# byuccl/coast

Measured on NVIDIA H100. Metric: protected-kernel throughput (MB/s voted output), sha256 TMR, higher is better.
Workload: dtype u32

## Files before the change

### coast_b200/csrc/coast_rt.c

```c
#define _GNU_SOURCE
#include "../../include/coast_rt.h"
#include "xmr_args.h"
#include "xmr_geom.h"

#include <cuda.h>
#include <ctype.h>
#include <dlfcn.h>
#include <sched.h>
#include <stdarg.h>
#include <stdio.h>
#include <stdlib.h>
#include <string.h>
#include <sys/syscall.h>
#include <unistd.h>

extern const unsigned char coast_kernels_cubin[];

__attribute__((weak)) uint32_t TMR_ERROR_CNT = 0;
__attribute__((weak)) uint64_t __SYNC_COUNT = 0;
__attribute__((weak)) void FAULT_DETECTED_DWC(void) {
    fprintf(stderr, "coast_rt: DWC mismatch detected -> FAULT_DETECTED_DWC -> abort()\n");
    abort();
}

#define DRV_FUNCS(X)                                                                                         \
    X(cuInit, (unsigned int))                                                                                \
    X(cuDeviceGet, (CUdevice*, int))                                                                         \
    X(cuDeviceGetAttribute, (int*, CUdevice_attribute, CUdevice))                                            \
    X(cuDeviceGetPCIBusId, (char*, int, CUdevice))                                                           \
    X(cuPointerGetAttribute, (void*, CUpointer_attribute, CUdeviceptr))                                      \
    X(cuDevicePrimaryCtxRetain, (CUcontext*, CUdevice))                                                      \
    X(cuDevicePrimaryCtxRelease_v2, (CUdevice))                                                              \
    X(cuCtxSetCurrent, (CUcontext))                                                                          \
    X(cuCtxGetCurrent, (CUcontext*))                                                                         \
    X(cuModuleLoadData, (CUmodule*, const void*))                                                            \
    X(cuModuleUnload, (CUmodule))                                                                            \
    X(cuModuleGetFunction, (CUfunction*, CUmodule, const char*))                                             \
    X(cuFuncSetAttribute, (CUfunction, CUfunction_attribute, int))                                           \
    X(cuOccupancyMaxActiveBlocksPerMultiprocessor, (int*, CUfunction, int, size_t))                          \
    X(cuLaunchKernel, (CUfunction, unsigned, unsigned, unsigned, unsigned, unsigned, unsigned, unsigned,     \
                       CUstream, void**, void**))                                                            \
    X(cuMemAlloc_v2, (CUdeviceptr*, size_t))                                                                 \
    X(cuMemFree_v2, (CUdeviceptr))                                                                           \
    X(cuMemPoolCreate, (CUmemoryPool*, const CUmemPoolProps*))                                               \
    X(cuMemPoolDestroy, (CUmemoryPool))                                                                      \
    X(cuMemPoolSetAttribute, (CUmemoryPool, CUmemPool_attribute, void*))                                     \
    X(cuMemAllocFromPoolAsync, (CUdeviceptr*, size_t, CUmemoryPool, CUstream))                               \
    X(cuMemFreeAsync, (CUdeviceptr, CUstream))                                                               \
    X(cuMemcpyHtoDAsync_v2, (CUdeviceptr, const void*, size_t, CUstream))                                    \
    X(cuMemcpyDtoHAsync_v2, (void*, CUdeviceptr, size_t, CUstream))                                          \
    X(cuMemcpyDtoDAsync_v2, (CUdeviceptr, CUdeviceptr, size_t, CUstream))                                    \
    X(cuMemsetD8Async, (CUdeviceptr, unsigned char, size_t, CUstream))                                       \
    X(cuMemHostAlloc, (void**, size_t, unsigned int))                                                        \
    X(cuMemFreeHost, (void*))                                                                                \
    X(cuStreamCreate, (CUstream*, unsigned int))                                                             \
    X(cuStreamDestroy_v2, (CUstream))                                                                        \
    X(cuStreamSynchronize, (CUstream))                                                                       \
    X(cuEventCreate, (CUevent*, unsigned int))                                                               \
    X(cuEventRecord, (CUevent, CUstream))                                                                    \
    X(cuEventDestroy_v2, (CUevent))                                                                          \
    X(cuStreamWaitEvent, (CUstream, CUevent, unsigned int))                                                  \
    X(cuGetErrorString, (CUresult, const char**))                                                            \
    X(cuIpcGetMemHandle, (CUipcMemHandle*, CUdeviceptr))                                                     \
    X(cuIpcOpenMemHandle_v2, (CUdeviceptr*, CUipcMemHandle, unsigned int))                                   \
    X(cuIpcCloseMemHandle, (CUdeviceptr))                                                                    \
    X(cuTensorMapEncodeTiled, (CUtensorMap*, CUtensorMapDataType, cuuint32_t, void*, const cuuint64_t*,      \
                               const cuuint64_t*, const cuuint32_t*, const cuuint32_t*, CUtensorMapInterleave, \
                               CUtensorMapSwizzle, CUtensorMapL2promotion, CUtensorMapFloatOOBfill))

#define X(name, args) static CUresult(CUDAAPI* p_##name) args;
DRV_FUNCS(X)
#undef X

typedef struct {
    uintptr_t base;
    cuuint64_t dim[3], stride[2];
    cuuint32_t box[3], rank;
    CUtensorMapDataType dtype;
    CUtensorMapSwizzle swz;
    CUtensorMapL2promotion l2;
    int in_scratch;
} map_desc;
_Static_assert(sizeof(map_desc) == 80, "map_desc has no padding");

typedef struct { CUdeviceptr p; size_t cap; } dev_buf;
typedef struct { CUstream s; dev_buf in, out, aux, stat, rows, sc; } host_slot;

#define MAX_FN 128
static struct {
    int inited;
    void* libcuda;
    int device;
    CUdevice dev;
    CUcontext ctx;
    CUmodule mod;
    int sm_count;
    CUdeviceptr counters;
    CUdeviceptr peer_counters;
    uint64_t* h_counters;
    struct { char name[64]; CUfunction fn; int ctas_per_sm; unsigned smem; } fns[MAX_FN];
    int n_fns;
    char err[512];
    uint32_t def_nc, def_flags; int def_set;
    host_slot slot[3];
    dev_buf h_b; CUevent ev_b;
    CUmemoryPool pool;
    int numa_node;
    int busy;
    struct { map_desc key; CUtensorMap map; } tmaps[16];
    int n_tmaps, tmap_next;
    unsigned warned_store_votes;
    int host_path_default;
    const char* last_host_path;
} G;

static int enter(void);
static void leave(void) { __atomic_store_n(&G.busy, 0, __ATOMIC_RELEASE); }

static int fail(int code, const char* fmt, ...) {
    va_list ap; va_start(ap, fmt);
    vsnprintf(G.err, sizeof G.err, fmt, ap);
    va_end(ap);
    return code;
}
static int enter(void) {
    if (__atomic_exchange_n(&G.busy, 1, __ATOMIC_ACQUIRE)) {
        return COAST_ERR_BUSY;
    }
    return COAST_OK;
}
#define ENTER() do { int e_ = enter(); if (e_) return e_; } while (0)
#define LEAVE(rc) do { int l_ = (rc); leave(); return l_; } while (0)
static int drv_fail(CUresult r, const char* what) {
    const char* s = NULL;
    if (p_cuGetErrorString) p_cuGetErrorString(r, &s);
    return fail(-(int)r, "%s: CUDA error %d (%s)", what, (int)r, s ? s : "?");
}
#define DRV(call) do { CUresult r_ = (call); if (r_ != CUDA_SUCCESS) return drv_fail(r_, #call); } while (0)

const char* coast_last_error(void) { return G.err; }
const char* coast_version(void) { return "coast_rt 0.1 (sm_90a)"; }

static int bind_driver(void) {
    if (G.libcuda) return COAST_OK;
    void* h = dlopen("libcuda.so.1", RTLD_NOW | RTLD_GLOBAL);
    if (!h) h = dlopen("libcuda.so", RTLD_NOW | RTLD_GLOBAL);
    if (!h) return fail(COAST_ERR_NO_DRIVER, "libcuda.so.1 not found (%s): no GPU driver on this machine; "
                                              "libcoast_rt has no CPU fallback", dlerror());
#define X(name, args)                                                                 \
    *(void**)(&p_##name) = dlsym(h, #name);                                           \
    if (!p_##name) { dlclose(h); return fail(COAST_ERR_NO_DRIVER, "libcuda lacks %s", #name); }
    DRV_FUNCS(X)
#undef X
    G.libcuda = h;
    return COAST_OK;
}


#ifndef MPOL_PREFERRED
#define MPOL_PREFERRED 1
#endif
static int parse_cpulist(const char* s, cpu_set_t* set) {
    int n = 0;
    CPU_ZERO(set);
    while (*s) {
        while (*s == ',' || isspace((unsigned char)*s)) ++s;
        if (!isdigit((unsigned char)*s)) break;
        char* e; long a = strtol(s, &e, 10), b = a;
        if (*e == '-') b = strtol(e + 1, &e, 10);
        for (long c = a; c <= b && c < CPU_SETSIZE; ++c) { CPU_SET((int)c, set); ++n; }
        s = e;
    }
    return n;
}
static void numa_bind_to_gpu(void) {
    G.numa_node = -1;
    const char* env = getenv("COAST_NUMA_BIND");
    if (env && !strcmp(env, "0")) return;
    char bdf[32] = {0}, path[128], buf[4096];
    if (p_cuDeviceGetPCIBusId(bdf, (int)sizeof bdf - 1, G.dev) != CUDA_SUCCESS) return;
    for (char* c = bdf; *c; ++c) *c = (char)tolower((unsigned char)*c);
    snprintf(path, sizeof path, "/sys/bus/pci/devices/%s/numa_node", bdf);
    FILE* f = fopen(path, "r"); if (!f) return;
    int node = -1; if (fscanf(f, "%d", &node) != 1) node = -1; fclose(f);
    if (node < 0 || node >= 1024) return;
    snprintf(path, sizeof path, "/sys/devices/system/node/node%d/cpulist", node);
    f = fopen(path, "r"); if (!f) return;
    size_t got = fread(buf, 1, sizeof buf - 1, f); fclose(f); buf[got] = 0;
    cpu_set_t want, cur, both;
    if (!parse_cpulist(buf, &want)) return;
    if (sched_getaffinity(0, sizeof cur, &cur)) return;
    CPU_AND(&both, &want, &cur);
    if (!CPU_COUNT(&both)) return;
    if (sched_setaffinity(0, sizeof both, &both)) return;
    unsigned long mask[16]; memset(mask, 0, sizeof mask);
    mask[node / (8 * sizeof(unsigned long))] |= 1ul << (node % (8 * sizeof(unsigned long)));
    syscall(SYS_set_mempolicy, MPOL_PREFERRED, mask, (unsigned long)(8 * sizeof mask));
    G.numa_node = node;
}
int coast_numa_node(void) { return G.inited ? G.numa_node : -1; }

static int ensure_ctx(void) {
    if (!G.inited) return fail(COAST_ERR_NOT_INIT, "coast_init() has not been called");
    CUcontext cur = NULL;
    p_cuCtxGetCurrent(&cur);
    if (cur != G.ctx) DRV(p_cuCtxSetCurrent(G.ctx));
// ... 213 lines not shown
    return kernel == COAST_K_QSORT ? unit_bytes : coast_out_bytes_per_unit(kernel);
}
static uint64_t in_bytes_per_unit(const coast_launch_desc* d) {
    if (!known_kernel(d->kernel)) return 0;
    return KINFO[d->kernel].in_bytes == IN_UNIT_BYTES ? d->unit_bytes : KINFO[d->kernel].in_bytes;
}
static uint64_t aux_bytes_per_unit(const coast_launch_desc* d) {
    return known_kernel(d->kernel) && (d->mode & COAST_AES_KEY_PER_UNIT) ? KINFO[d->kernel].key_bytes : 0;
}

static int encode_map(const map_desc* want, CUdeviceptr scratch, int cached, CUtensorMap* map) {
    map_desc m = *want;
    if (m.in_scratch) { m.base += scratch; m.in_scratch = 0; }
    if (cached)
        for (int i = 0; i < G.n_tmaps; ++i)
            if (!memcmp(&G.tmaps[i].key, &m, sizeof m)) { *map = G.tmaps[i].map; return COAST_OK; }
    static const cuuint32_t estr[3] = { 1, 1, 1 };
    DRV(p_cuTensorMapEncodeTiled(map, m.dtype, m.rank, (void*)m.base, m.dim, m.stride, m.box, estr, CU_TENSOR_MAP_INTERLEAVE_NONE,
                                 m.swz, m.l2, CU_TENSOR_MAP_FLOAT_OOB_FILL_NONE));
    if (cached) {
        const int n_slots = (int)(sizeof G.tmaps / sizeof G.tmaps[0]);
        int k = G.n_tmaps < n_slots ? G.n_tmaps++ : (G.tmap_next++ % n_slots);
        G.tmaps[k].key = m; G.tmaps[k].map = *map;
    }
    return COAST_OK;
}

typedef struct {
    unsigned es;
    int batched, grouped, bt;
    uint64_t P;
    uint64_t rows;
    int b_rows_k;
    uint32_t b_rows;
    int scaled, rowwise;
} mm_shape;

typedef struct launch_plan launch_plan;
struct launch_plan {
    char name[64];
    unsigned block, smem;
    uint64_t ctas;
    unsigned waves;
    unsigned cluster;
    int n_maps, cache_maps;
    map_desc map[2];
    size_t scratch;
    size_t scratch_per_cta;
    int scratch_as_aux;
    int (*prepass)(const launch_plan* L, const coast_launch_desc* d, CUdeviceptr scratch, CUstream s);
    mm_shape mm;
    size_t grp_off;
    unsigned grp_tm, grp_tiles_n;
};

static void plan_ring(launch_plan* L, xmr_args* a, unsigned tile_rows, unsigned row_bytes, unsigned pack, CUtensorMapSwizzle swz) {
    L->ctas = (a->n_units + tile_rows - 1) / tile_rows;
    L->waves = 1;
    a->n_tiles = (unsigned)L->ctas;
    L->n_maps = 1; L->cache_maps = 1;
    map_desc* m = &L->map[0];
    m->dtype = CU_TENSOR_MAP_DATA_TYPE_UINT32; m->rank = 2; m->base = (uintptr_t)a->in;
    m->dim[0] = m->box[0] = (row_bytes << pack) / 4u;
    m->dim[1] = a->n_units >> pack;
    m->stride[0] = row_bytes << pack;
    m->box[1] = (tile_rows / xmr_ring_loads(tile_rows)) >> pack;
    m->swz = swz; m->l2 = CU_TENSOR_MAP_L2_PROMOTION_L2_128B;
}

static void plan_wg_map(map_desc* m, CUtensorMapDataType dtype, unsigned esize, uintptr_t base, int in_scratch, uint32_t K,
                        uint32_t rows, unsigned planes, unsigned box_rows) {
    m->dtype = dtype; m->rank = planes > 1 ? 3 : 2; m->base = base; m->in_scratch = in_scratch;
    m->dim[0] = K; m->dim[1] = rows; m->dim[2] = planes;
    m->stride[0] = (cuuint64_t)K * esize; m->stride[1] = (cuuint64_t)rows * K * esize;
    m->box[0] = 128u / esize; m->box[1] = box_rows; m->box[2] = planes;
    m->swz = CU_TENSOR_MAP_SWIZZLE_128B; m->l2 = CU_TENSOR_MAP_L2_PROMOTION_L2_256B;
}

static int mm_rows_fit(const mm_shape* m) { return m->rows < (1ull << 31) && m->P * m->b_rows < (1ull << 31); }

static int mm_bit_refused(const coast_launch_desc* d, uint32_t bit) {
    if (!(d->mode & bit) || is_matmul(d->kernel)) return COAST_OK;
    const char* what = bit == COAST_MM_BATCHED ? "COAST_MM_BATCHED: batched products exist"
                     : bit == COAST_MM_GROUPED ? "COAST_MM_GROUPED: grouped products exist" : "COAST_MM_B_TRANSPOSED: a transposed B exists";
    return fail(COAST_ERR_BAD_ARG, "%s for MM_U32, GEMM_TF32 and GEMM_BF16 only, plus GEMM_FP8 (kernel %u)", what, d->kernel);
}
static int mm_scale_check(const coast_launch_desc* d) {
    const uint32_t bits = d->mode & (COAST_MM_SCALE_TENSOR | COAST_MM_SCALE_ROWWISE);
    if (!bits) return COAST_OK;
    const char* what = bits == COAST_MM_SCALE_TENSOR ? "COAST_MM_SCALE_TENSOR" : "COAST_MM_SCALE_ROWWISE";
    if (d->kernel != COAST_K_GEMM_FP8)
        return fail(COAST_ERR_BAD_ARG, "%s: scaled products exist for GEMM_FP8 only (kernel %u)",
                    bits == (COAST_MM_SCALE_TENSOR | COAST_MM_SCALE_ROWWISE) ? "COAST_MM_SCALE_TENSOR / COAST_MM_SCALE_ROWWISE" : what, d->kernel);
    if (bits == (COAST_MM_SCALE_TENSOR | COAST_MM_SCALE_ROWWISE))
        return fail(COAST_ERR_BAD_ARG, "COAST_MM_SCALE_TENSOR and COAST_MM_SCALE_ROWWISE cannot be combined: one scale layout per launch");
    if (!d->d_scale_a || !d->d_scale_b)
        return fail(COAST_ERR_BAD_ARG, "%s: d_scale_a and d_scale_b must point to the scales of A and B", what);
    if (((uintptr_t)d->d_scale_a) & 3u) return fail(COAST_ERR_BAD_ARG, "%s: d_scale_a must be 4-byte aligned", what);
    if (bits == COAST_MM_SCALE_ROWWISE && (((uintptr_t)d->d_scale_b) & 7u))
        return fail(COAST_ERR_BAD_ARG, "COAST_MM_SCALE_ROWWISE: d_scale_b must be 8-byte aligned (column scales are read in pairs)");
    return COAST_OK;
}
static int mm_check(const coast_launch_desc* d, mm_shape* m) {
    int rc;
    memset(m, 0, sizeof *m);
    if ((rc = mm_bit_refused(d, COAST_MM_BATCHED)) || (rc = mm_bit_refused(d, COAST_MM_GROUPED)) ||
// ... 106 lines not shown
                                           "4..4096 (got %u)", d->unit_bytes);
        if ((((uintptr_t)d->d_in) & 3u) || (((uintptr_t)d->d_out) & 3u))
            return fail(COAST_ERR_BAD_ARG, "COAST_UNIT_OFFSETS: quicksort's d_in and d_out must be 4-byte aligned");
    }
    if (d->n_units >= (1ull << 32)) return fail(COAST_ERR_BAD_ARG, "COAST_UNIT_OFFSETS: n_units must be below 2^32");
    if (!d->d_aux || (((uintptr_t)d->d_aux) & 7u))
        return fail(COAST_ERR_BAD_ARG, "COAST_UNIT_OFFSETS: d_aux must point to n_units + 1 8-byte aligned uint64_t offsets");
    return COAST_OK;
}

static int prepass_ragged(const launch_plan* L, const coast_launch_desc* d, CUdeviceptr scratch, CUstream s) {
    (void)L;
    DRV(p_cuMemsetD8Async(scratch, 0, XMR_RAGGED_PERM, s));
    const void* off = d->d_aux;
    unsigned long long n = d->n_units;
    unsigned int bound = d->unit_bytes;
    unsigned int kind = d->kernel == COAST_K_SHA256 ? XMR_RAGGED_COST_SHA : d->kernel == COAST_K_QSORT ? XMR_RAGGED_COST_QSORT
                                                                                                       : XMR_RAGGED_COST_CRC;
    const uint64_t ctas = (n + XMR_CTA_THREADS - 1) / XMR_CTA_THREADS, cap = (uint64_t)G.sm_count * 8u;
    const unsigned grid = (unsigned)(ctas < cap ? ctas : cap);
    void* params[] = { &off, &n, &bound, &kind, &scratch };
    int rc = launch_small("xmr_ragged_hist", grid, XMR_CTA_THREADS, params, s); if (rc) return rc;
    void* params_scan[] = { &off, &scratch };
    rc = launch_small("xmr_ragged_scan", 1, XMR_RAGGED_SCAN_THREADS, params_scan, s); if (rc) return rc;
    return launch_small("xmr_ragged_scatter", grid, XMR_CTA_THREADS, params, s);
}

static int run_plan(const launch_plan* L, const coast_launch_desc* d, xmr_args* a, CUstream stream) {
    CUfunction fn; int occ = 1;
    int rc = get_fn(L->name, L->smem, L->block, &fn, &occ); if (rc) return rc;
    const uint64_t cap = (uint64_t)G.sm_count * (unsigned)occ * L->waves;
    unsigned grid = (unsigned)(L->waves && L->ctas > cap ? cap : L->ctas);
    grid -= grid % L->cluster;
    const size_t bytes = L->scratch + (size_t)grid * L->scratch_per_cta;
    CUdeviceptr scratch = 0;
    if (bytes) DRV(p_cuMemAllocFromPoolAsync(&scratch, bytes, G.pool, stream));
    if (L->scratch_per_cta || L->scratch_as_aux) a->aux = (const void*)scratch;
    CUtensorMap maps[2];
    rc = L->prepass ? L->prepass(L, d, scratch, stream) : COAST_OK;
    for (int i = 0; i < L->n_maps && !rc; ++i) rc = encode_map(&L->map[i], scratch, L->cache_maps, &maps[i]);
    const void* ro = d->d_rows; const void* sa = d->d_scale_a; const void* sb = d->d_scale_b;
    CUdeviceptr grp = scratch + L->grp_off;
    if (!rc && L->mm.grouped && L->grp_tm)
        rc = prepass_group_scan(L, d, grp, d->kernel != COAST_K_MM_U32 ? &maps[0] : NULL, stream);
    if (!rc) {
        void* params[7] = { a };
        int n_params = 1;
        for (int i = 0; i < L->n_maps; ++i) params[n_params++] = &maps[i];
        if (L->mm.grouped) { params[n_params++] = &ro; params[n_params++] = &grp; }
        if (L->mm.scaled) { params[n_params++] = &sa; params[n_params++] = &sb; }
        if (d->flags & COAST_F_VERBOSE)
            fprintf(stderr, "coast_rt: %s grid=%u block=%u smem=%u units=%llu\n", L->name, grid, L->block, L->smem,
                    (unsigned long long)d->n_units);
        CUresult r = p_cuLaunchKernel(fn, grid, 1, 1, L->block, 1, 1, L->smem, stream, params, NULL);
        if (r != CUDA_SUCCESS) rc = drv_fail(r, "cuLaunchKernel");
    }
    if (scratch) p_cuMemFreeAsync(scratch, stream);
    return rc;
}

static int launch_impl(const coast_launch_desc* d, void* stream) {
    int rc = ensure_ctx(); if (rc) return rc;
    if (!d) return fail(COAST_ERR_BAD_ARG, "null descriptor");
    if (!known_kernel(d->kernel)) return fail(COAST_ERR_BAD_ARG, "unknown kernel id %u", d->kernel);
    if (d->num_clones < 1 || d->num_clones > 3) return fail(COAST_ERR_BAD_ARG, "num_clones must be 1, 2 (DWC) or 3 (TMR)");
    const int ragged = (d->mode & COAST_UNIT_OFFSETS) != 0;
    if (ragged && (rc = ragged_check(d))) return rc;
    mm_shape m;
    if ((rc = mm_check(d, &m))) return rc;
    if (d->n_units == 0) return COAST_OK;
    if (!d->d_in || !d->d_out) return fail(COAST_ERR_BAD_ARG, "null device buffer");
    const uint32_t nc = d->num_clones;
    const uint32_t upw = xmr_units_per_warp(nc);
    const int inj = d->plan && d->plan->mode != COAST_PLAN_NONE;

    xmr_args a; memset(&a, 0, sizeof a);
    a.in = d->d_in; a.out = d->d_out; a.aux = d->d_aux;
    a.n_units = d->n_units; a.unit_base = d->unit_base;
    a.counters = (unsigned long long*)(G.peer_counters ? G.peer_counters : G.counters);
    a.status = (unsigned char*)d->d_status;
    a.unit_bytes = d->unit_bytes; a.flags = d->flags; a.mode = d->mode & ~(COAST_MM_BATCHED | COAST_MM_GROUPED | COAST_MM_B_TRANSPOSED |
                                                                      COAST_MM_SCALE_TENSOR | COAST_MM_SCALE_ROWWISE);
    if (m.rowwise) a.mode |= XMR_MODE_SCALE_ROWWISE;
    a.M = d->M; a.N = d->N; a.K = d->K;
    memcpy(a.key, d->key, 16);
    if (inj) {
        a.plan_mode = d->plan->mode; a.seed_lo = d->plan->seed_lo; a.seed_hi = d->plan->seed_hi;
        a.threshold = d->plan->threshold; a.plan_table = (const unsigned int*)d->plan->d_table;
        if (a.plan_mode == COAST_PLAN_TABLE && !a.plan_table) return fail(COAST_ERR_BAD_ARG, "TABLE plan without d_table");
        if (a.plan_mode > COAST_PLAN_TABLE) return fail(COAST_ERR_BAD_ARG, "unknown fault plan mode %u", a.plan_mode);
    }
    a.n_sites = coast_fault_sites(d->kernel, d->unit_bytes, d->K);
    const int store_votes = store_votes_wanted(d->flags) && nc > 1;
    if (store_votes && !store_votes_built(d->kernel)) {
        const char* strict = getenv("COAST_STRICT_FLAGS");
        if (strict && strcmp(strict, "0"))
            return fail(COAST_ERR_UNSUPPORTED, "-noMemReplication / -storeDataSync: the %s kernel has no in-loop store votes "
                                               "(COAST_STRICT_FLAGS is set)", KINFO[d->kernel].name);
        if (!(G.warned_store_votes & (1u << d->kernel))) {
            G.warned_store_votes |= 1u << d->kernel;
            fprintf(stderr, "coast_rt: WARNING: -noMemReplication / -storeDataSync are NOT honoured by the %s kernel: it has no in-loop "
                            "store votes and runs the default sync set (SoR-exit votes only).  COAST_STRICT_FLAGS=1 makes this an error.\n",
                    KINFO[d->kernel].name);
        }
    }
    if (store_votes && store_votes_built(d->kernel)) a.flags |= XMR_F_STORE_VOTES;

    launch_plan L; memset(&L, 0, sizeof L);
    L.block = XMR_CTA_THREADS; L.waves = 4; L.cluster = 1;
    const int aligned16 = (((uintptr_t)d->d_in) & 15u) == 0;
    const int ring_ok = d->unit_bytes == 64 && aligned16 && d->n_units < 0x7FFFFF00ull && !store_votes;
    L.mm = m;
    if (is_matmul(d->kernel)) {
        const char* fam = d->kernel == COAST_K_MM_U32 ? "MM" : "GEMM";
        if (!d->d_aux || !d->M || !d->N || !d->K) return fail(COAST_ERR_BAD_ARG, "%s needs A (d_in), B (d_aux) and M,N,K", fam);
        if (!m.batched && !m.grouped && d->n_units != (uint64_t)d->M * d->N) return fail(COAST_ERR_BAD_ARG, "%s: n_units must be M*N", fam);
    }
    switch (d->kernel) {
    case COAST_K_SHA256:
        if (((uintptr_t)d->d_out) & 15u) return fail(COAST_ERR_BAD_ARG, "SHA output must be 16-byte aligned");
        if (ragged) {
            snprintf(L.name, sizeof L.name, "xmr_sha256_var_inj%d_nc%u", inj, nc);
        } else if (!ring_ok) {
            snprintf(L.name, sizeof L.name, "xmr_sha256_gen_nc%u_inj%d", nc, inj);
        } else if (nc == 3 && !(d->flags & COAST_F_INTERLEAVE)) {
            snprintf(L.name, sizeof L.name, "xmr_sha256_b64_seg_nc3_inj%d", inj);
            L.block = XMR_SHA_SEG_THREADS; L.smem = xmr_sha_seg_smem();
            plan_ring(&L, &a, XMR_SHA_SEG_TILE_ROWS, 64, 0, CU_TENSOR_MAP_SWIZZLE_64B);
        } else {
            snprintf(L.name, sizeof L.name, "xmr_sha256_b64_nc%u_inj%d", nc, inj);
            L.smem = xmr_sha_smem(nc);
            plan_ring(&L, &a, xmr_sha_tile_rows(nc), 64, 0, CU_TENSOR_MAP_SWIZZLE_64B);
        }
        break;
    case COAST_K_CRC16:
        if (ragged) {
            snprintf(L.name, sizeof L.name, "xmr_crc16_var_inj%d_nc%u", inj, nc);
            break;
        }
        if (d->unit_bytes < 1 || d->unit_bytes > 255) return fail(COAST_ERR_BAD_ARG, "crc16 length is an unsigned char (1..255)");
        if (ring_ok) {
            snprintf(L.name, sizeof L.name, "xmr_crc16_b64_nc%u_inj%d", nc, inj);
            L.block = xmr_crc_threads(nc); L.smem = xmr_crc_smem(nc);
            plan_ring(&L, &a, xmr_crc_tile_rows(nc), 64, 0, CU_TENSOR_MAP_SWIZZLE_64B);
        } else {
            snprintf(L.name, sizeof L.name, "xmr_crc16_gen_nc%u_inj%d", nc, inj);
        }
        break;
    case COAST_K_AES128: {
        const int dec = (d->mode & COAST_AES_DECRYPT) != 0, perkey = (d->mode & COAST_AES_KEY_PER_UNIT) != 0;
        if (perkey && !d->d_aux) return fail(COAST_ERR_BAD_ARG, "per-unit keys need d_aux");
        if (!aligned16 || (((uintptr_t)d->d_out) & 15u)) return fail(COAST_ERR_BAD_ARG, "AES buffers must be 16-byte aligned");
        if (perkey && (((uintptr_t)d->d_aux) & 15u)) return fail(COAST_ERR_BAD_ARG, "AES per-unit keys must be 16-byte aligned");
        if (d->n_units >= 0x7FFFFF00ull) return fail(COAST_ERR_UNSUPPORTED, "AES: at most 2^31 - 257 blocks per launch (split the batch)");
        static const char* const stem[4] = { "xmr_aes128_enc", "xmr_aes128_dec", "xmr_aes128_enck", "xmr_aes128_deck" };
        snprintf(L.name, sizeof L.name, "%s_nc%u_inj%d", stem[dec + 2 * perkey], nc, inj);
        L.block = XMR_AES_THREADS; L.smem = xmr_aes_smem(dec);
        const unsigned tile_rows = xmr_aes_tile_rows(nc), box_rows = tile_rows / xmr_ring_loads(tile_rows);
        unsigned pack = d->n_units % 16u == 0 ? 4u : d->n_units % 4u == 0 ? 2u : 0u;
        while (pack && box_rows % (1u << pack)) pack -= 2u;
        a.mode = (a.mode & ~(XMR_MODE_AES_ROWPACK_MASK << XMR_MODE_AES_ROWPACK_SHIFT)) | (pack << XMR_MODE_AES_ROWPACK_SHIFT);
        plan_ring(&L, &a, tile_rows, 16, pack, CU_TENSOR_MAP_SWIZZLE_NONE);
        break;
    }
    case COAST_K_MM_U32: {
        const char* path = getenv("COAST_MM_PATH");
        const int aligned = aligned16 && !(((uintptr_t)d->d_aux) & 15u) && !(((uintptr_t)d->d_out) & 15u);
        const int tiles_ok = !store_votes && aligned;
        const char* variant = "";
        int bt_name = m.bt;
        if (tiles_ok && (!path || !strcmp(path, "tc")) && (m.grouped || d->M % XMR_WG_BM == 0) && d->N % xmr_mmtc_bn(1) == 0 &&
            d->K % XMR_MMTC_BK == 0) {
            const unsigned bn = xmr_mmtc_bn(nc);
            variant = "_tc";
            bt_name = m.bt && inj;
            L.block = XMR_WG_THREADS; L.smem = xmr_mmtc_smem(nc);
            L.ctas = mm_row_tiles(&m, XMR_WG_BM) * (d->N / bn); L.waves = 1;
            L.scratch = ((size_t)m.rows * d->K + (size_t)m.P * d->K * d->N) * 4u;
            L.prepass = prepass_split_limbs;
            L.grp_tm = XMR_WG_BM; L.grp_tiles_n = d->N / bn;
// ... 639 lines not shown
```

### coast_b200/csrc/xmr_common.cuh

```cuda
#pragma once
#include <cuda.h>
#include <cuda_runtime.h>
#include <stdint.h>
#include "../../include/coast_rt.h"
#include "xmr_args.h"
#include "xmr_geom.h"

namespace xmr {

struct u4 { uint32_t x, y, z, w; };

__device__ __forceinline__ u4 philox4x32_10(uint32_t c0, uint32_t c1, uint32_t c2, uint32_t c3, uint32_t k0, uint32_t k1) {
#pragma unroll
    for (int r = 0; r < 10; ++r) {
        uint32_t hi0 = __umulhi(0xD2511F53u, c0), lo0 = 0xD2511F53u * c0;
        uint32_t hi1 = __umulhi(0xCD9E8D57u, c2), lo1 = 0xCD9E8D57u * c2;
        uint32_t n0 = hi1 ^ c1 ^ k0, n2 = hi0 ^ c3 ^ k1;
        c0 = n0; c1 = lo1; c2 = n2; c3 = lo0;
        k0 += 0x9E3779B9u; k1 += 0xBB67AE85u;
    }
    return u4{c0, c1, c2, c3};
}

struct Fault { bool active; uint32_t replica, site, bit; };
// ... 131 lines not shown
            }
        } else if (NC == 2) {
            dwc += bad ? 1u : 0u;
        }
        if (NC > 1 && bad && gunit < first) first = gunit;
        if (status) status[gunit - base] = (unsigned char)(NC > 1 ? (bad > 255u ? 255u : bad) : 0u);
    }
    __device__ __forceinline__ void flush(unsigned long long* ctr) {
        uint32_t e = __reduce_add_sync(0xFFFFFFFFu, errors);
        uint32_t d = __reduce_add_sync(0xFFFFFFFFu, dwc);
        uint32_t s = __reduce_add_sync(0xFFFFFFFFu, syncs);
        uint32_t j = __reduce_add_sync(0xFFFFFFFFu, injected);
        uint32_t fhi = __reduce_min_sync(0xFFFFFFFFu, (uint32_t)(first >> 32));
        uint32_t flo = __reduce_min_sync(0xFFFFFFFFu, (uint32_t)(first >> 32) == fhi ? (uint32_t)first : 0xFFFFFFFFu);
        if ((threadIdx.x & 31) == 0) {
            if (e) atomicAdd_system(ctr + XMR_CTR_ERRORS, (unsigned long long)e);
            if (d) atomicAdd_system(ctr + XMR_CTR_DWC, (unsigned long long)d);
            if (s) atomicAdd_system(ctr + XMR_CTR_SYNCS, (unsigned long long)s);
            if (j) atomicAdd_system(ctr + XMR_CTR_INJECTED, (unsigned long long)j);
            unsigned long long f = ((unsigned long long)fhi << 32) | flo;
            if (f != ~0ull) atomicMin_system(ctr + XMR_CTR_FIRST, f);
        }
    }
};

__device__ __forceinline__ uint32_t smem_u32(const void* p) { return (uint32_t)__cvta_generic_to_shared(p); }

__device__ __forceinline__ void mbar_init(uint64_t* bar, uint32_t count) {
    asm volatile("mbarrier.init.shared::cta.b64 [%0], %1;" ::"r"(smem_u32(bar)), "r"(count));
}
__device__ __forceinline__ void fence_barrier_init() { asm volatile("fence.mbarrier_init.release.cluster;" ::: "memory"); }
__device__ __forceinline__ void fence_proxy_async() { asm volatile("fence.proxy.async.shared::cta;" ::: "memory"); }
__device__ __forceinline__ void mbar_arrive_expect_tx(uint64_t* bar, uint32_t bytes) {
    asm volatile("mbarrier.arrive.expect_tx.shared::cta.b64 _, [%0], %1;" ::"r"(smem_u32(bar)), "r"(bytes) : "memory");
}
__device__ __forceinline__ void mbar_wait(uint64_t* bar, uint32_t parity) {
    asm volatile(
        "{\n\t.reg .pred p;\n\t"
        "WAIT_%=:\n\t"
        "mbarrier.try_wait.parity.shared::cta.b64 p, [%0], %1;\n\t"
        "@p bra DONE_%=;\n\t"
        "bra WAIT_%=;\n\t"
        "DONE_%=:\n\t}" ::"r"(smem_u32(bar)), "r"(parity) : "memory");
}
__device__ __forceinline__ void tma_load_2d(void* smem_dst, const CUtensorMap* map, uint64_t* bar, int c0, int c1) {
    asm volatile(
        "cp.async.bulk.tensor.2d.shared::cluster.global.tile.mbarrier::complete_tx::bytes [%0], [%1, {%3, %4}], [%2];"
        ::"r"(smem_u32(smem_dst)), "l"(map), "r"(smem_u32(bar)), "r"(c0), "r"(c1) : "memory");
}
__device__ __forceinline__ void tma_prefetch_desc(const CUtensorMap* map) {
    asm volatile("prefetch.tensormap [%0];" ::"l"(map) : "memory");
}

template <int TILE_ROWS, int ROW_BYTES>
struct TileRing {
    static constexpr int LOADS = (int)xmr_ring_loads(TILE_ROWS);
    static constexpr int BOX_ROWS = TILE_ROWS / LOADS;
    static_assert(TILE_ROWS % LOADS == 0 && BOX_ROWS <= 256, "tile must split into equal TMA boxes");
    static constexpr uint32_t TILE_BYTES = (uint32_t)TILE_ROWS * ROW_BYTES;
    static constexpr uint32_t STAGE_STRIDE = xmr_ring_stride(TILE_ROWS, ROW_BYTES);
    static constexpr uint32_t SMEM_BYTES = xmr_ring_smem(XMR_STAGES, TILE_ROWS, ROW_BYTES, XMR_RING_TAIL);
    static_assert(XMR_STAGES * sizeof(uint64_t) <= XMR_RING_TAIL, "the full barriers fit behind the tiles");
    uint8_t* tiles;
    uint64_t* full;
    const CUtensorMap* tmap;
    uint32_t pack_shift = 0;
    __device__ __forceinline__ void init(uint8_t* smem, const CUtensorMap* map, uint32_t row_pack_shift = 0) {
        pack_shift = row_pack_shift;
        tiles = smem;
        full = reinterpret_cast<uint64_t*>(smem + XMR_STAGES * STAGE_STRIDE);
        tmap = map;
        if (threadIdx.x == 0) {
            tma_prefetch_desc(map);
#pragma unroll
            for (int s = 0; s < XMR_STAGES; ++s) mbar_init(&full[s], 1);
            fence_barrier_init();
        }
        __syncthreads();
    }
    __device__ __forceinline__ void issue(uint32_t stage, uint32_t tile) {
        if (threadIdx.x == 0) {
            mbar_arrive_expect_tx(&full[stage], TILE_BYTES);
#pragma unroll
            for (int l = 0; l < LOADS; ++l)
                tma_load_2d(tiles + stage * STAGE_STRIDE + l * BOX_ROWS * ROW_BYTES, tmap, &full[stage], 0,
                            (int)((tile * TILE_ROWS + l * BOX_ROWS) >> pack_shift));
        }
    }
    __device__ __forceinline__ const uint8_t* wait(uint32_t it) {
        mbar_wait(&full[it & 1u], (it >> 1) & 1u);
        return tiles + (it & 1u) * STAGE_STRIDE;
    }
};

}
```

### coast_b200/csrc/xmr_sha256.cuh

```cuda
#pragma once
#include "xmr_common.cuh"

namespace xmr {

__device__ __forceinline__ constexpr uint32_t sha_k(int i) {
    constexpr uint32_t K[64] = {
        0x428a2f98u, 0x71374491u, 0xb5c0fbcfu, 0xe9b5dba5u, 0x3956c25bu, 0x59f111f1u, 0x923f82a4u, 0xab1c5ed5u,
        0xd807aa98u, 0x12835b01u, 0x243185beu, 0x550c7dc3u, 0x72be5d74u, 0x80deb1feu, 0x9bdc06a7u, 0xc19bf174u,
        0xe49b69c1u, 0xefbe4786u, 0x0fc19dc6u, 0x240ca1ccu, 0x2de92c6fu, 0x4a7484aau, 0x5cb0a9dcu, 0x76f988dau,
        0x983e5152u, 0xa831c66du, 0xb00327c8u, 0xbf597fc7u, 0xc6e00bf3u, 0xd5a79147u, 0x06ca6351u, 0x14292967u,
        0x27b70a85u, 0x2e1b2138u, 0x4d2c6dfcu, 0x53380d13u, 0x650a7354u, 0x766a0abbu, 0x81c2c92eu, 0x92722c85u,
        0xa2bfe8a1u, 0xa81a664bu, 0xc24b8b70u, 0xc76c51a3u, 0xd192e819u, 0xd6990624u, 0xf40e3585u, 0x106aa070u,
        0x19a4c116u, 0x1e376c08u, 0x2748774cu, 0x34b0bcb5u, 0x391c0cb3u, 0x4ed8aa4au, 0x5b9cca4fu, 0x682e6ff3u,
        0x748f82eeu, 0x78a5636fu, 0x84c87814u, 0x8cc70208u, 0x90befffau, 0xa4506cebu, 0xbef9a3f7u, 0xc67178f2u};
    return K[i];
}

constexpr uint32_t SHA_SITES_PER_BLOCK = 536u;

__device__ __forceinline__ uint32_t rotr(uint32_t v, int n) { return __funnelshift_r(v, v, n); }
__device__ __forceinline__ uint32_t bswap(uint32_t v) { return __byte_perm(v, 0u, 0x0123u); }

__constant__ uint32_t sha_one = 1u;

// ... 224 lines not shown
            uint32_t m[16];
            if ((al & 15u) == 0 && blk * 64u + 64u <= len) {
#pragma unroll
                for (int c = 0; c < 4; ++c) {
                    const uint4 q = __ldg(reinterpret_cast<const uint4*>(msg + blk * 64u) + c);
                    m[4 * c + 0] = bswap(q.x); m[4 * c + 1] = bswap(q.y); m[4 * c + 2] = bswap(q.z); m[4 * c + 3] = bswap(q.w);
                }
            } else {
#pragma unroll
                for (int w = 0; w < 16; ++w) {
                    const uint32_t p = blk * 64u + 4u * w;
                    if ((al & 3u) == 0 && p + 4u <= len) m[w] = bswap(__ldg(reinterpret_cast<const uint32_t*>(msg + p)));
                    else m[w] = (sha_padded_byte(msg, len, p) << 24) | (sha_padded_byte(msg, len, p + 1) << 16) |
                                (sha_padded_byte(msg, len, p + 2) << 8) | sha_padded_byte(msg, len, p + 3);
                }
            }
            if (blk == nblk - 1) {
                m[14] = len >> 29;
                m[15] = len << 3;
            }
            uint32_t fs = (INJECT && fsite / SHA_SITES_PER_BLOCK == blk) ? fsite % SHA_SITES_PER_BLOCK : 0xFFFFFFFFu;
            if (!sv) {
                sha_compress<INJECT>(st, m, fs, fmask);
            } else {
                const uint32_t lo = blk * 64u, nmsg = len > lo ? (len - lo < 64u ? len - lo : 64u) : 0u;
#pragma unroll
                for (int w = 0; w < 16; ++w) {
                    const uint32_t nb = nmsg > 4u * w ? (nmsg - 4u * w < 4u ? nmsg - 4u * w : 4u) : 0u;
                    sv_bad += store_vote_bytes<NC>(m[w], nb, lane, majority);
                }
                sv_bad += sha_compress_sv<NC, INJECT>(st, m, fs, fmask, lane, majority);
            }
        }
        if (!sv) {
            sha_vote_store<NC>(st, static_cast<uint8_t*>(a.out), local, gunit, valid, lane, a.flags, tally);
        } else {
            uint32_t o[8], bad = 0;
#pragma unroll
            for (int i = 0; i < 8; ++i) { Voted v = vote_u32<NC, 1>(st[i], majority); o[i] = bswap(v.vote); bad += v.bad; }
            if (valid && Lanes<NC>::voter(lane)) {
                uint4* dst = reinterpret_cast<uint4*>(static_cast<uint8_t*>(a.out) + local * 32ull);
                dst[0] = make_uint4(o[0], o[1], o[2], o[3]);
                dst[1] = make_uint4(o[4], o[5], o[6], o[7]);
                tally.unit_exit<NC>(bad + sv_bad, len + 720u * nblk + 32u, a.flags, gunit);
            }
        }
    }
    tally.flush(a.counters);
}

constexpr int SEG_THREADS = XMR_SHA_SEG_THREADS, SEG_GROUPS = SEG_THREADS / 96, SEG_TU = SEG_GROUPS * 32;
constexpr uint32_t SEG_EXCH_WORDS = 2 * 8 * 32;

template <bool INJECT>
__device__ __forceinline__ void sha256_b64_seg_body(const xmr_args& a, const CUtensorMap* tmap) {
    using Ring = TileRing<SEG_TU, 64>;
    static_assert(SEG_TU == XMR_SHA_SEG_TILE_ROWS && Ring::SMEM_BYTES <= xmr_sha_seg_exch_offset() &&
                  xmr_sha_seg_exch_offset() + 2u * SEG_GROUPS * SEG_EXCH_WORDS * 4u <= xmr_sha_seg_smem(),
                  "ring and exchange buffer fit the launch's shared memory");
    extern __shared__ __align__(1024) uint8_t smem_raw[];
    Ring ring;
    ring.init(smem_raw, tmap);
    uint32_t* exch = reinterpret_cast<uint32_t*>(smem_raw + xmr_sha_seg_exch_offset());
    const int tid = threadIdx.x, lane = tid & 31, warp = tid >> 5;
    const int g = warp / 3, r = warp - 3 * g;
    const int ul = g * 32 + lane;
    const uint32_t n_tiles = a.n_tiles;
    const bool majority = a.flags & COAST_F_MAJORITY_VOTER;
    uint32_t tile = blockIdx.x;
    if (tile < n_tiles) ring.issue(0, tile);
    Tally tally(a);
    uint32_t it = 0;
    for (; tile < n_tiles; tile += gridDim.x, ++it) {
        const uint32_t next = tile + gridDim.x;
        if (next < n_tiles) ring.issue((it + 1u) & 1u, next);
        const uint8_t* base = ring.wait(it);
        uint32_t m[16];
        const uint8_t* row = base + ul * 64;
        const int sw = (ul >> 1) & 3;
#pragma unroll
        for (int c = 0; c < 4; ++c) {
            uint4 q = *reinterpret_cast<const uint4*>(row + ((c ^ sw) << 4));
            m[4 * c + 0] = bswap(q.x); m[4 * c + 1] = bswap(q.y); m[4 * c + 2] = bswap(q.z); m[4 * c + 3] = bswap(q.w);
        }
        __syncthreads();
        const unsigned long long local = (unsigned long long)tile * SEG_TU + ul;
        const bool valid = local < a.n_units;
        uint32_t fs0 = 0xFFFFFFFFu, fs1 = 0xFFFFFFFFu, fmask = 0u;
        if (INJECT) {
            Fault f = fault_for_unit(a, 3, valid ? local : 0ull, [](uint32_t) { return 32u; });
            if (f.active && valid) {
                if (r == 0) tally.injected++;
                if ((int)f.replica == r) {
                    fmask = 1u << f.bit;
                    if (f.site < SHA_SITES_PER_BLOCK) fs0 = f.site; else fs1 = f.site - SHA_SITES_PER_BLOCK;
                }
            }
        }
        uint32_t st[8];
        sha_init(st);
        sha_compress<INJECT>(st, m, fs0, fmask);
#pragma unroll
        for (int i = 0; i < 16; ++i) m[i] = 0u;
        m[0] = 0x80000000u; m[15] = 512u;
        sha_compress<INJECT, true>(st, m, fs1, fmask);

        uint32_t* ex = exch + ((it & 1u) * SEG_GROUPS + g) * SEG_EXCH_WORDS;
        if (r > 0) {
#pragma unroll
            for (int i = 0; i < 8; ++i) ex[((r - 1) * 8 + i) * 32 + lane] = st[i];
        }
        if (g == 0) asm volatile("bar.sync 1, 96;" ::: "memory");
        else if (g == 1) asm volatile("bar.sync 2, 96;" ::: "memory");
        else if (g == 2) asm volatile("bar.sync 3, 96;" ::: "memory");
        else asm volatile("bar.sync 4, 96;" ::: "memory");
        if (r == 0) {
            uint32_t o[8], bad = 0;
#pragma unroll
            for (int i = 0; i < 8; ++i) {
                const uint32_t x = st[i], r1 = ex[i * 32 + lane], r2 = ex[(8 + i) * 32 + lane];
                const uint32_t e01 = __vcmpeq4(x, r1), e02 = __vcmpeq4(x, r2);
                const uint32_t v = majority ? ((x & r1) | (x & r2) | (r1 & r2)) : ((x & e01) | (r2 & ~e01));
                bad += __popc(~(e01 & e02)) >> 3;
                o[i] = bswap(v);
            }
            if (valid) {
                uint4* dst = reinterpret_cast<uint4*>(static_cast<uint8_t*>(a.out) + local * 32ull);
                dst[0] = make_uint4(o[0], o[1], o[2], o[3]);
                dst[1] = make_uint4(o[4], o[5], o[6], o[7]);
                tally.unit_exit<3>(bad, 32u, a.flags, a.unit_base + local);
            }
        }
    }
    tally.flush(a.counters);
}

}

#define XMR_SHA_B64_KERNEL(NC, INJ)                                                                      \
    extern "C" __global__ void __launch_bounds__(XMR_CTA_THREADS)                                        \
    xmr_sha256_b64_nc##NC##_inj##INJ(const __grid_constant__ xmr_args a, const __grid_constant__ CUtensorMap tmap) { \
        xmr::sha256_b64_body<NC, INJ != 0>(a, &tmap);                                                    \
    }
#define XMR_SHA_GEN_KERNEL(NC, INJ)                                                                      \
    extern "C" __global__ void __launch_bounds__(XMR_CTA_THREADS)                                        \
    xmr_sha256_gen_nc##NC##_inj##INJ(const __grid_constant__ xmr_args a) {                               \
        xmr::sha256_gen_body<NC, INJ != 0>(a);                                                           \
    }
XMR_SHA_B64_KERNEL(1, 0) XMR_SHA_B64_KERNEL(2, 0) XMR_SHA_B64_KERNEL(3, 0)
XMR_SHA_B64_KERNEL(1, 1) XMR_SHA_B64_KERNEL(2, 1) XMR_SHA_B64_KERNEL(3, 1)
XMR_SHA_GEN_KERNEL(1, 0) XMR_SHA_GEN_KERNEL(2, 0) XMR_SHA_GEN_KERNEL(3, 0)
XMR_SHA_GEN_KERNEL(1, 1) XMR_SHA_GEN_KERNEL(2, 1) XMR_SHA_GEN_KERNEL(3, 1)

#define XMR_SHA_B64_SEG_KERNEL(INJ)                                                                      \
    extern "C" __global__ void __launch_bounds__(xmr::SEG_THREADS)                                       \
    xmr_sha256_b64_seg_nc3_inj##INJ(const __grid_constant__ xmr_args a, const __grid_constant__ CUtensorMap tmap) { \
        xmr::sha256_b64_seg_body<INJ != 0>(a, &tmap);                                                    \
    }
XMR_SHA_B64_SEG_KERNEL(0) XMR_SHA_B64_SEG_KERNEL(1)
```

Baseline: 92110.

## Add PDL launch, per-warp empty-barrier ring release, and fast-path voter for SHA seg

Launches the segmented SHA-256 TMR kernel with programmatic dependent launch, so the next kernel's prologue can overlap the tail of the previous one. Replaces the CTA-wide __syncthreads after reading a tile with per-warp arrivals on new empty mbarriers, and has a dedicated thread wait on them before issuing the next TMA load. It also adds a fast voter path: when all three replicas agree across the warp, it writes the digest directly and calls a non-inlined byte-wise vote only on mismatch. The risks are extra mbarrier traffic, a correctness dependency on the PDL wait ordering, and different register pressure.

```diff
diff --git a/coast_b200/csrc/coast_rt.c b/coast_b200/csrc/coast_rt.c
--- a/coast_b200/csrc/coast_rt.c
+++ b/coast_b200/csrc/coast_rt.c
@@ -71,6 +71,7 @@
 #define X(name, args) static CUresult(CUDAAPI* p_##name) args;
 DRV_FUNCS(X)
 #undef X
+static CUresult(CUDAAPI* p_cuLaunchKernelEx)(const CUlaunchConfig*, CUfunction, void**, void**);
 
 typedef struct {
     uintptr_t base;
@@ -152,6 +153,7 @@
     if (!p_##name) { dlclose(h); return fail(COAST_ERR_NO_DRIVER, "libcuda lacks %s", #name); }
     DRV_FUNCS(X)
 #undef X
+    *(void**)(&p_cuLaunchKernelEx) = dlsym(h, "cuLaunchKernelEx");
     G.libcuda = h;
     return COAST_OK;
 }
@@ -471,6 +473,7 @@
     mm_shape mm;
     size_t grp_off;
     unsigned grp_tm, grp_tiles_n;
+    int pdl;
 };
 
 static void plan_ring(launch_plan* L, xmr_args* a, unsigned tile_rows, unsigned row_bytes, unsigned pack, CUtensorMapSwizzle swz) {
@@ -683,8 +686,21 @@
         if (d->flags & COAST_F_VERBOSE)
             fprintf(stderr, "coast_rt: %s grid=%u block=%u smem=%u units=%llu\n", L->name, grid, L->block, L->smem,
                     (unsigned long long)d->n_units);
-        CUresult r = p_cuLaunchKernel(fn, grid, 1, 1, L->block, 1, 1, L->smem, stream, params, NULL);
-        if (r != CUDA_SUCCESS) rc = drv_fail(r, "cuLaunchKernel");
+        const char* pdl_env = getenv("COAST_PDL");
+        if (L->pdl && p_cuLaunchKernelEx && !(pdl_env && !strcmp(pdl_env, "0"))) {
+            CUlaunchAttribute attr; memset(&attr, 0, sizeof attr);
+            attr.id = CU_LAUNCH_ATTRIBUTE_PROGRAMMATIC_STREAM_SERIALIZATION;
+            attr.value.programmaticStreamSerializationAllowed = 1;
+            CUlaunchConfig cfg; memset(&cfg, 0, sizeof cfg);
+            cfg.gridDimX = grid; cfg.gridDimY = 1; cfg.gridDimZ = 1;
+            cfg.blockDimX = L->block; cfg.blockDimY = 1; cfg.blockDimZ = 1;
+            cfg.sharedMemBytes = L->smem; cfg.hStream = stream; cfg.attrs = &attr; cfg.numAttrs = 1;
+            CUresult r = p_cuLaunchKernelEx(&cfg, fn, params, NULL);
+            if (r != CUDA_SUCCESS) rc = drv_fail(r, "cuLaunchKernelEx");
+        } else {
+            CUresult r = p_cuLaunchKernel(fn, grid, 1, 1, L->block, 1, 1, L->smem, stream, params, NULL);
+            if (r != CUDA_SUCCESS) rc = drv_fail(r, "cuLaunchKernel");
+        }
     }
     if (scratch) p_cuMemFreeAsync(scratch, stream);
     return rc;
@@ -756,7 +772,7 @@
             snprintf(L.name, sizeof L.name, "xmr_sha256_gen_nc%u_inj%d", nc, inj);
         } else if (nc == 3 && !(d->flags & COAST_F_INTERLEAVE)) {
             snprintf(L.name, sizeof L.name, "xmr_sha256_b64_seg_nc3_inj%d", inj);
-            L.block = XMR_SHA_SEG_THREADS; L.smem = xmr_sha_seg_smem();
+            L.block = XMR_SHA_SEG_THREADS; L.smem = xmr_sha_seg_smem(); L.pdl = 1;
             plan_ring(&L, &a, XMR_SHA_SEG_TILE_ROWS, 64, 0, CU_TENSOR_MAP_SWIZZLE_64B);
         } else {
             snprintf(L.name, sizeof L.name, "xmr_sha256_b64_nc%u_inj%d", nc, inj);
diff --git a/coast_b200/csrc/xmr_common.cuh b/coast_b200/csrc/xmr_common.cuh
--- a/coast_b200/csrc/xmr_common.cuh
+++ b/coast_b200/csrc/xmr_common.cuh
@@ -207,7 +207,7 @@
     asm volatile("prefetch.tensormap [%0];" ::"l"(map) : "memory");
 }
 
-template <int TILE_ROWS, int ROW_BYTES>
+template <int TILE_ROWS, int ROW_BYTES, int RELEASERS = 0>
 struct TileRing {
     static constexpr int LOADS = (int)xmr_ring_loads(TILE_ROWS);
     static constexpr int BOX_ROWS = TILE_ROWS / LOADS;
@@ -215,26 +215,31 @@
     static constexpr uint32_t TILE_BYTES = (uint32_t)TILE_ROWS * ROW_BYTES;
     static constexpr uint32_t STAGE_STRIDE = xmr_ring_stride(TILE_ROWS, ROW_BYTES);
     static constexpr uint32_t SMEM_BYTES = xmr_ring_smem(XMR_STAGES, TILE_ROWS, ROW_BYTES, XMR_RING_TAIL);
-    static_assert(XMR_STAGES * sizeof(uint64_t) <= XMR_RING_TAIL, "the full barriers fit behind the tiles");
+    static_assert(2 * XMR_STAGES * sizeof(uint64_t) <= XMR_RING_TAIL, "the full and empty barriers fit behind the tiles");
     uint8_t* tiles;
     uint64_t* full;
+    uint64_t* empty;
     const CUtensorMap* tmap;
     uint32_t pack_shift = 0;
     __device__ __forceinline__ void init(uint8_t* smem, const CUtensorMap* map, uint32_t row_pack_shift = 0) {
         pack_shift = row_pack_shift;
         tiles = smem;
         full = reinterpret_cast<uint64_t*>(smem + XMR_STAGES * STAGE_STRIDE);
+        empty = full + XMR_STAGES;
         tmap = map;
         if (threadIdx.x == 0) {
             tma_prefetch_desc(map);
 #pragma unroll
-            for (int s = 0; s < XMR_STAGES; ++s) mbar_init(&full[s], 1);
+            for (int s = 0; s < XMR_STAGES; ++s) {
+                mbar_init(&full[s], 1);
+                if (RELEASERS > 0) mbar_init(&empty[s], RELEASERS);
+            }
             fence_barrier_init();
         }
         __syncthreads();
     }
     __device__ __forceinline__ void issue(uint32_t stage, uint32_t tile) {
-        if (threadIdx.x == 0) {
+        if (RELEASERS > 0 || threadIdx.x == 0) {
             mbar_arrive_expect_tx(&full[stage], TILE_BYTES);
 #pragma unroll
             for (int l = 0; l < LOADS; ++l)
@@ -246,6 +251,17 @@
         mbar_wait(&full[it & 1u], (it >> 1) & 1u);
         return tiles + (it & 1u) * STAGE_STRIDE;
     }
+    __device__ __forceinline__ void release(uint32_t it, int lane) {
+        static_assert(RELEASERS > 0, "a ring without empty barriers is released with __syncthreads");
+        __syncwarp();
+        if (lane == 0) asm volatile("mbarrier.arrive.shared::cta.b64 _, [%0];" ::"r"(smem_u32(&empty[it & 1u])) : "memory");
+    }
+    __device__ __forceinline__ void wait_empty(uint32_t it) {
+        mbar_wait(&empty[it & 1u], (it >> 1) & 1u);
+    }
 };
 
-}
+__device__ __forceinline__ void grid_dependency_wait() { asm volatile("griddepcontrol.wait;" ::: "memory"); }
+__device__ __forceinline__ void grid_launch_dependents() { asm volatile("griddepcontrol.launch_dependents;" ::: "memory"); }
+
+}
diff --git a/coast_b200/csrc/xmr_sha256.cuh b/coast_b200/csrc/xmr_sha256.cuh
--- a/coast_b200/csrc/xmr_sha256.cuh
+++ b/coast_b200/csrc/xmr_sha256.cuh
@@ -300,9 +300,24 @@
 constexpr int SEG_THREADS = XMR_SHA_SEG_THREADS, SEG_GROUPS = SEG_THREADS / 96, SEG_TU = SEG_GROUPS * 32;
 constexpr uint32_t SEG_EXCH_WORDS = 2 * 8 * 32;
 
+__device__ __noinline__ uint32_t seg_vote_bytes(const uint32_t* ex, int lane, bool majority, uint32_t* dst, uint32_t x0, uint32_t x1,
+                                                uint32_t x2, uint32_t x3, uint32_t x4, uint32_t x5, uint32_t x6, uint32_t x7) {
+    uint32_t bad = 0;
+#pragma unroll 1
+    for (int i = 0; i < 8; ++i) {
+        const uint32_t x = x0, r1 = ex[i * 32 + lane], r2 = ex[(8 + i) * 32 + lane];
+        const uint32_t e01 = __vcmpeq4(x, r1), e02 = __vcmpeq4(x, r2);
+        const uint32_t v = majority ? ((x & r1) | (x & r2) | (r1 & r2)) : ((x & e01) | (r2 & ~e01));
+        bad += __popc(~(e01 & e02)) >> 3;
+        if (dst) dst[i] = bswap(v);
+        x0 = x1; x1 = x2; x2 = x3; x3 = x4; x4 = x5; x5 = x6; x6 = x7;
+    }
+    return bad;
+}
+
 template <bool INJECT>
 __device__ __forceinline__ void sha256_b64_seg_body(const xmr_args& a, const CUtensorMap* tmap) {
-    using Ring = TileRing<SEG_TU, 64>;
+    using Ring = TileRing<SEG_TU, 64, SEG_THREADS / 32>;
     static_assert(SEG_TU == XMR_SHA_SEG_TILE_ROWS && Ring::SMEM_BYTES <= xmr_sha_seg_exch_offset() &&
                   xmr_sha_seg_exch_offset() + 2u * SEG_GROUPS * SEG_EXCH_WORDS * 4u <= xmr_sha_seg_smem(),
                   "ring and exchange buffer fit the launch's shared memory");
@@ -315,13 +330,18 @@
     const int ul = g * 32 + lane;
     const uint32_t n_tiles = a.n_tiles;
     const bool majority = a.flags & COAST_F_MAJORITY_VOTER;
+    grid_dependency_wait();
     uint32_t tile = blockIdx.x;
-    if (tile < n_tiles) ring.issue(0, tile);
+    if (tid == 32 && tile < n_tiles) ring.issue(0, tile);
     Tally tally(a);
     uint32_t it = 0;
     for (; tile < n_tiles; tile += gridDim.x, ++it) {
         const uint32_t next = tile + gridDim.x;
-        if (next < n_tiles) ring.issue((it + 1u) & 1u, next);
+        if (next >= n_tiles) grid_launch_dependents();
+        if (tid == 32 && next < n_tiles) {
+            if (it >= 1u) ring.wait_empty(it - 1u);
+            ring.issue((it + 1u) & 1u, next);
+        }
         const uint8_t* base = ring.wait(it);
         uint32_t m[16];
         const uint8_t* row = base + ul * 64;
@@ -331,7 +351,7 @@
             uint4 q = *reinterpret_cast<const uint4*>(row + ((c ^ sw) << 4));
             m[4 * c + 0] = bswap(q.x); m[4 * c + 1] = bswap(q.y); m[4 * c + 2] = bswap(q.z); m[4 * c + 3] = bswap(q.w);
         }
-        __syncthreads();
+        ring.release(it, lane);
         const unsigned long long local = (unsigned long long)tile * SEG_TU + ul;
         const bool valid = local < a.n_units;
         uint32_t fs0 = 0xFFFFFFFFu, fs1 = 0xFFFFFFFFu, fmask = 0u;
@@ -363,21 +383,21 @@
         else if (g == 2) asm volatile("bar.sync 3, 96;" ::: "memory");
         else asm volatile("bar.sync 4, 96;" ::: "memory");
         if (r == 0) {
-            uint32_t o[8], bad = 0;
-#pragma unroll
-            for (int i = 0; i < 8; ++i) {
-                const uint32_t x = st[i], r1 = ex[i * 32 + lane], r2 = ex[(8 + i) * 32 + lane];
-                const uint32_t e01 = __vcmpeq4(x, r1), e02 = __vcmpeq4(x, r2);
-                const uint32_t v = majority ? ((x & r1) | (x & r2) | (r1 & r2)) : ((x & e01) | (r2 & ~e01));
-                bad += __popc(~(e01 & e02)) >> 3;
-                o[i] = bswap(v);
-            }
-            if (valid) {
-                uint4* dst = reinterpret_cast<uint4*>(static_cast<uint8_t*>(a.out) + local * 32ull);
-                dst[0] = make_uint4(o[0], o[1], o[2], o[3]);
-                dst[1] = make_uint4(o[4], o[5], o[6], o[7]);
-                tally.unit_exit<3>(bad, 32u, a.flags, a.unit_base + local);
-            }
+            uint32_t diff = 0;
+#pragma unroll
+            for (int i = 0; i < 8; ++i) diff |= (st[i] ^ ex[i * 32 + lane]) | (st[i] ^ ex[(8 + i) * 32 + lane]);
+            uint8_t* dst = static_cast<uint8_t*>(a.out) + local * 32ull;
+            uint32_t bad = 0;
+            if (__all_sync(0xFFFFFFFFu, diff == 0u)) {
+                if (valid) {
+                    reinterpret_cast<uint4*>(dst)[0] = make_uint4(bswap(st[0]), bswap(st[1]), bswap(st[2]), bswap(st[3]));
+                    reinterpret_cast<uint4*>(dst)[1] = make_uint4(bswap(st[4]), bswap(st[5]), bswap(st[6]), bswap(st[7]));
+                }
+            } else {
+                bad = seg_vote_bytes(ex, lane, majority, valid ? reinterpret_cast<uint32_t*>(dst) : nullptr, st[0], st[1], st[2], st[3],
+                                     st[4], st[5], st[6], st[7]);
+            }
+            if (valid) tally.unit_exit<3>(bad, 32u, a.flags, a.unit_base + local);
         }
     }
     tally.flush(a.counters);
```

New measurement: 93600 (median of 6 runs). 1.6% higher.
